# epam/ai-dial-rag

Hardware: AMD Instinct MI355X
Metric: retrieval_qps_10Mx384 (higher is better)
Workload: dtype f32 (int8 MFMA filter with exact integer dot products and a rigorous error margin, every candidate the margin cannot exclude re-scored in f64 with the reference formula)

## Files before the change

ai-dial-rag_amd/csrc/vec_kernels.h:

```cpp
#pragma once
#include <hip/hip_runtime.h>
#include <stdint.h>

#include <type_traits>

namespace mir {

typedef __attribute__((ext_vector_type(8))) __bf16 bf16x8;
typedef __attribute__((ext_vector_type(16))) float f32x16;

constexpr int kTileRows = 32;
constexpr int kMaxList = 64;
constexpr int kListMargin = 8;
constexpr int kSortN = 8192;
constexpr double kScanSplitErr = 4.6e-5;
__host__ __device__ constexpr double scan_rel_err(int d) { return kScanSplitErr + 6.0e-8 * (d < 384 ? 384 : d); }

enum ScanKind { SCAN_IP = 0, SCAN_L2 = 1, SCAN_COS = 2 };


__device__ __forceinline__ uint32_t bf16_rne_bits(float x) {
    uint32_t u = __float_as_uint(x);
    if ((u & 0x7fffffffu) > 0x7f800000u) return 0x7fc0u;
    return (u + 0x7fffu + ((u >> 16) & 1u)) >> 16;
// ... 131 lines not shown
}

__device__ __forceinline__ float ref_row_norm(double s, float doc_sq32) {
    return doc_sq32 == __builtin_inff() ? __builtin_inff() : fmaxf((float)sqrt(s), 1e-8f);
}

template <typename T>
__global__ __launch_bounds__(256) void row_norms_kernel(const T *__restrict__ src, int64_t n, int d,
                                                        float *__restrict__ doc_sq,
                                                        float *__restrict__ inv_norm,
                                                        unsigned int *__restrict__ max_norm_bits) {
    int64_t row = (int64_t)blockIdx.x * 256 + threadIdx.x;
    float nrm = 0.f, res = 0.f, rel = 0.f;
    if (row < n) {
        const T *a = src + row * (int64_t)d;
        const float dsq = np_pairwise_sq<12>(a, d);
        doc_sq[row] = dsq;
        const double s = seq_sum_sq_f64(a, d);
        nrm = (float)sqrt(s);
        nrm = nrm * (1.0f + 1e-6f);
        inv_norm[row] = 1.0f / ref_row_norm(s, dsq);
        if (sizeof(T) == 4) {
            res = bf16_residual_norm(a, d);
            rel = res * inv_norm[row] * (1.0f + 1e-6f);
        }
    }
    for (int off = 32; off >= 1; off >>= 1) { res = fmaxf(res, __shfl_xor(res, off, 64)); rel = fmaxf(rel, __shfl_xor(rel, off, 64)); }
    if ((threadIdx.x & 63) == 0 && res > 0.f) { atomicMax(max_norm_bits + 2, __float_as_uint(res)); atomicMax(max_norm_bits + 3, __float_as_uint(rel)); }
    if (__ballot(!(nrm < __builtin_inff())) != 0ull && (threadIdx.x & 63) == 0) atomicOr(max_norm_bits + 1, 1u);
    for (int off = 32; off >= 1; off >>= 1) nrm = fmaxf(nrm, __shfl_xor(nrm, off, 64));
    if ((threadIdx.x & 63) == 0 && nrm > 0.f) atomicMax(max_norm_bits, __float_as_uint(nrm));
}

constexpr int kNormsLdsBytes = 64 * 1024;
__host__ __device__ inline int norms_row_stride(int d) { return d | 1; }
template <typename T>
__global__ __launch_bounds__(256) void row_norms_lds_kernel(const T *__restrict__ src, int64_t n, int d, int rows_per_wg,
                                                            float *__restrict__ doc_sq, float *__restrict__ inv_norm,
                                                            unsigned int *__restrict__ max_norm_bits) {
    extern __shared__ float norms_lds[];
    const int stride = norms_row_stride(d);
    const int64_t row0 = (int64_t)blockIdx.x * rows_per_wg;
    const int rows = (int)(n - row0 < rows_per_wg ? n - row0 : rows_per_wg);
    const T *base = src + row0 * (int64_t)d;
    const int total = rows * d;
    for (int e0 = threadIdx.x; e0 < total; e0 += 256 * 16) {
        T v[16];
#pragma unroll
        for (int u = 0; u < 16; ++u) {
            const int e = e0 + 256 * u;
            v[u] = e < total ? base[e] : T(0);
        }
        int r = e0 / d, c = e0 - r * d;
#pragma unroll
        for (int u = 0; u < 16; ++u) {
            if (e0 + 256 * u < total) norms_lds[r * stride + c] = (float)v[u];
            c += 256;
            while (c >= d) { c -= d; ++r; }
        }
    }
    __syncthreads();
    float nrm = 0.f, res = 0.f, rel = 0.f;
    const int rt = threadIdx.x & 127;
    const float *a = norms_lds + rt * stride;
    const int64_t row = row0 + rt;
    double s = 0.0;
    if (rt < rows) {
        if (threadIdx.x < 128) {
            doc_sq[row] = np_pairwise_sq<12>(a, d);
        } else {
            s = seq_sum_sq_f64(a, d);
        }
    }
    __syncthreads();
    if (rt < rows && threadIdx.x >= 128) {
        nrm = (float)sqrt(s);
        nrm = nrm * (1.0f + 1e-6f);
        inv_norm[row] = 1.0f / ref_row_norm(s, const_cast<const volatile float *>(doc_sq)[row]);
        if (sizeof(T) == 4) {
            res = bf16_residual_norm(a, d);
            rel = res * inv_norm[row] * (1.0f + 1e-6f);
        }
    }
    for (int off = 32; off >= 1; off >>= 1) { res = fmaxf(res, __shfl_xor(res, off, 64)); rel = fmaxf(rel, __shfl_xor(rel, off, 64)); }
    if ((threadIdx.x & 63) == 0 && res > 0.f) { atomicMax(max_norm_bits + 2, __float_as_uint(res)); atomicMax(max_norm_bits + 3, __float_as_uint(rel)); }
    if (__ballot(!(nrm < __builtin_inff())) != 0ull && (threadIdx.x & 63) == 0) atomicOr(max_norm_bits + 1, 1u);
    for (int off = 32; off >= 1; off >>= 1) nrm = fmaxf(nrm, __shfl_xor(nrm, off, 64));
    if ((threadIdx.x & 63) == 0 && nrm > 0.f) atomicMax(max_norm_bits, __float_as_uint(nrm));
}


__global__ __launch_bounds__(64) void prep_queries_kernel(const double *__restrict__ q, int b, int d, int ksteps,
                                                          int ngroups, uint4 *__restrict__ qsplit,
                                                          double *__restrict__ q_sq,
                                                          double *__restrict__ q_norm,
                                                          unsigned long long *__restrict__ gthr, int gthr_words) {
    int lane = threadIdx.x;
    int blk = blockIdx.x;
    if (gthr && blk * 64 + lane < gthr_words) gthr[blk * 64 + lane] = 0;
    if (blk < ngroups * ksteps) {
        int s = blk % ksteps;
        int g = blk / ksteps;
        int qi = 32 * g + (lane & 31);
        int col0 = 16 * s + 8 * (lane >> 5);
        uint32_t hi[8], lo[8];
#pragma unroll
        for (int j = 0; j < 8; ++j) {
            float x = (qi < b && col0 + j < d) ? (float)q[(int64_t)qi * d + col0 + j] : 0.f;
            split_bf16(x, hi[j], lo[j]);
        }
        qsplit[((int64_t)blk * 2 + 0) * 64 + lane] = pack8(hi);
        qsplit[((int64_t)blk * 2 + 1) * 64 + lane] = pack8(lo);
    } else {
        int qi = blk - ngroups * ksteps;
        if (qi >= b) return;
        double s = 0.0;
        for (int j = lane; j < d; j += 64) {
            double x = q[(int64_t)qi * d + j];
            s += x * x;
        }
        s = wave_sum(s);
        if (lane == 0) {
            q_sq[qi] = s;
            q_norm[qi] = sqrt(s);
        }
    }
}


template <int STRIDE = 256>
__device__ __forceinline__ void list_insert(uint64_t *list, int klist, int tid, uint64_t key, uint64_t &minkey,
                                            int &minpos) {
    list[minpos * STRIDE + tid] = key;
    uint64_t m = ~0ull;
    int mp = 0;
    for (int p0 = 0; p0 < klist; p0 += 8) {
        uint64_t x[8];
#pragma unroll
        for (int j = 0; j < 8; ++j) x[j] = (p0 + j < klist) ? list[(p0 + j) * STRIDE + tid] : ~0ull;
#pragma unroll
        for (int j = 0; j < 8; ++j) {
            if (x[j] < m) {
                m = x[j];
                mp = p0 + j;
            }
        }
    }
    minkey = m;
    minpos = mp;
}

template <int KIND>
__device__ __forceinline__ void tile_epilogue(const f32x16 &acc_m, const f32x16 &acc_c, const float4 (&ax)[4],
                                              uint32_t row0, uint32_t n_rows, uint64_t *list, int klist, int tid,
                                              uint64_t &minkey, int &minpos) {
    float v[16];
    uint32_t mask = 0;
    const float vmin = key_value(minkey);
    const bool open = minkey == 0;
#pragma unroll
    for (int r = 0; r < 16; ++r) {
        const int g = r >> 2, i = r & 3;
        const float dot = acc_m[r] + acc_c[r];
        float x;
        if (KIND == SCAN_IP) {
            x = dot;
        } else {
            const float a = (i == 0) ? ax[g].x : (i == 1) ? ax[g].y : (i == 2) ? ax[g].z : ax[g].w;
            x = (KIND == SCAN_L2) ? fmaf(2.0f, dot, -a) : dot * a;
        }
        x = (x == x) ? x + 0.0f : -__builtin_inff();
        v[r] = x;
        const uint32_t row = row0 + 8 * g + i;
        if (row < n_rows && (open || x >= vmin)) mask |= 1u << r;
    }
    while (mask) {
        const int r = __builtin_ctz(mask);
        mask &= mask - 1;
        float x = v[0];
#pragma unroll
        for (int j = 1; j < 16; ++j) x = (r == j) ? v[j] : x;
        const uint32_t row = row0 + 8 * (r >> 2) + (r & 3);
        const uint64_t key = make_key(x, row);
        if (key > minkey) list_insert(list, klist, tid, key, minkey, minpos);
    }
}

template <int KSTEPS, int KIND>
__global__ __launch_bounds__(256, 1) void scan_topk_kernel(const uint4 *__restrict__ docs,
                                                           const float *__restrict__ aux,
                                                           const uint4 *__restrict__ qsplit, uint32_t n_rows,
                                                           uint32_t n_tiles, int nq, int klist,
                                                           uint64_t *__restrict__ part) {
    extern __shared__ __attribute__((aligned(16))) unsigned char smem[];
    uint64_t *list = reinterpret_cast<uint64_t *>(smem);
    uint64_t *stage = list + klist * 256;

    constexpr int R = KSTEPS < 8 ? KSTEPS : 8;
    static_assert(KSTEPS % R == 0, "ring slot must be static across tiles");
    constexpr int TILE_U4 = KSTEPS * 128;

    const int tid = threadIdx.x;
    const int lane = tid & 63;
    const int h = lane >> 5;
    const int qj = lane & 31;
    const uint32_t wave_global = blockIdx.x * 4 + (tid >> 6);
    const uint32_t total_waves = gridDim.x * 4;

    for (int p = 0; p < klist; ++p) list[p * 256 + tid] = 0;
    uint64_t minkey = 0;
    int minpos = 0;

    if (wave_global < n_tiles) {
        bf16x8 qh[KSTEPS], ql[KSTEPS];
#pragma unroll
        for (int s = 0; s < KSTEPS; ++s) {
            qh[s] = __builtin_bit_cast(bf16x8, qsplit[(s * 2 + 0) * 64 + lane]);
            ql[s] = __builtin_bit_cast(bf16x8, qsplit[(s * 2 + 1) * 64 + lane]);
        }

        uint32_t t = wave_global;
        const uint4 *tp = docs + (size_t)t * TILE_U4 + lane;
        uint4 bh[R], bl[R];
#pragma unroll
        for (int i = 0; i < R; ++i) {
            bh[i] = tp[(2 * i + 0) * 64];
            bl[i] = tp[(2 * i + 1) * 64];
        }

        while (true) {
            const uint32_t tn = t + total_waves;
            const bool more = tn < n_tiles;
            const uint4 *np = docs + (size_t)(more ? tn : t) * TILE_U4 + lane;

            float4 ax[4];
            if (KIND != SCAN_IP) {
                const float4 *ap = reinterpret_cast<const float4 *>(aux + (size_t)t * kTileRows);
#pragma unroll
                for (int g = 0; g < 4; ++g) ax[g] = ap[2 * g + h];
            }

            f32x16 acc_m = {0}, acc_c = {0};
#pragma unroll
            for (int ks = 0; ks < KSTEPS; ++ks) {
                const int slot = ks % R;
                bf16x8 ah = __builtin_bit_cast(bf16x8, bh[slot]);
                bf16x8 al = __builtin_bit_cast(bf16x8, bl[slot]);
                acc_m = __builtin_amdgcn_mfma_f32_32x32x16_bf16(ah, qh[ks], acc_m, 0, 0, 0);
                acc_c = __builtin_amdgcn_mfma_f32_32x32x16_bf16(ah, ql[ks], acc_c, 0, 0, 0);
                acc_c = __builtin_amdgcn_mfma_f32_32x32x16_bf16(al, qh[ks], acc_c, 0, 0, 0);
                if (ks + R < KSTEPS) {
                    bh[slot] = tp[(2 * (ks + R) + 0) * 64];
                    bl[slot] = tp[(2 * (ks + R) + 1) * 64];
                } else {
                    bh[slot] = np[(2 * (ks + R - KSTEPS) + 0) * 64];
                    bl[slot] = np[(2 * (ks + R - KSTEPS) + 1) * 64];
                }
                __builtin_amdgcn_sched_barrier(0);
            }

            if (qj < nq) tile_epilogue<KIND>(acc_m, acc_c, ax, t * kTileRows + 4 * h, n_rows, list, klist, tid, minkey, minpos);
            if (!more) break;
            t = tn;
            tp = np;
        }
    }

    __syncthreads();
    for (int i = tid; i < 32 * klist; i += 256) stage[i] = 0;
    __syncthreads();
    for (int p = 0; p < klist; ++p) {
        const uint64_t key = list[p * 256 + tid];
        if (key == 0) continue;
        int rank = 0;
        for (int l = 0; l < 8; ++l) {
            const int t2 = 64 * (l >> 1) + 32 * (l & 1) + qj;
            for (int p2 = 0; p2 < klist; ++p2) rank += (list[p2 * 256 + t2] > key) ? 1 : 0;
        }
        if (rank < klist) stage[qj * klist + rank] = key;
    }
    __syncthreads();
    uint64_t *out = part + (size_t)blockIdx.x * 32 * klist;
    for (int i = tid; i < 32 * klist; i += 256) out[i] = stage[i];
}

constexpr int kB128Pending = 4;

__device__ __forceinline__ void glds16_b128(const void *gsrc, uint32_t lds_byte_addr) {
    uint32_t keep;
    asm volatile(
        "s_mov_b32 %0, m0\n\ts_mov_b32 m0, %2\n\ts_nop 0\n\tglobal_load_lds_dwordx4 %1, off nt\n\ts_mov_b32 m0, %0"
        : "=&s"(keep)
        : "v"(gsrc), "s"(lds_byte_addr)
        : "memory");
}
__device__ __forceinline__ void glds4_b32(const void *gsrc, uint32_t lds_byte_addr) {
    uint32_t keep;
    asm volatile(
        "s_mov_b32 %0, m0\n\ts_mov_b32 m0, %2\n\ts_nop 0\n\tglobal_load_lds_dword %1, off\n\ts_mov_b32 m0, %0"
        : "=&s"(keep)
        : "v"(gsrc), "s"(lds_byte_addr)
        : "memory");
}
__device__ __forceinline__ void glds4_b32_sv(const void *gbase_uniform, uint32_t lane_byte_off, uint32_t lds_byte_addr) {
    uint32_t keep;
    asm volatile(
        "s_mov_b32 %0, m0\n\ts_mov_b32 m0, %3\n\ts_nop 0\n\tglobal_load_lds_dword %1, %2\n\ts_mov_b32 m0, %0"
        : "=&s"(keep)
        : "v"(lane_byte_off), "s"(gbase_uniform), "s"(lds_byte_addr)
        : "memory");
}
__device__ __forceinline__ uint32_t lds_addr_of(const void *p) {
    return (uint32_t)(uintptr_t)(const __attribute__((address_space(3))) void *)p;
}

template <int STRIDE = 256>
__device__ __forceinline__ void drain_candidates(uint32_t mask, const float (&v)[16], uint32_t row0, uint64_t *list,
                                                 int klist, int tid, uint64_t &minkey, int &minpos, int &pending) {
    while (__any(mask != 0)) {
        if (mask) {
            const int r = __builtin_ctz(mask);
            mask &= mask - 1;
            float x = v[0];
#pragma unroll
            for (int j = 1; j < 16; ++j) {
                float c = v[j];
                asm volatile("" : "+v"(c));
                x = (r == j) ? c : x;
            }
            x = (x == x) ? x + 0.0f : -__builtin_inff();
            const uint64_t key = make_key(x, row0 + 8 * (r >> 2) + (r & 3));
            if (key > minkey) {
                list[(klist + pending) * STRIDE + tid] = key;
                ++pending;
            }
        }
        if (__any(pending == kB128Pending)) {
            for (int i = 0; i < kB128Pending; ++i) {
                if (i < pending) {
                    const uint64_t key = list[(klist + i) * STRIDE + tid];
                    if (key > minkey) list_insert<STRIDE>(list, klist, tid, key, minkey, minpos);
                }
            }
            pending = 0;
        }
    }
}

template <int KIND>
__global__ __launch_bounds__(256, 1) void scan_topk_generic_kernel(const uint4 *__restrict__ docs,
                                                                   const float *__restrict__ aux,
                                                                   const uint4 *__restrict__ qsplit,
                                                                   int ksteps, uint32_t n_rows,
                                                                   uint32_t n_tiles, int nq, int klist,
                                                                   uint64_t *__restrict__ part) {
    extern __shared__ __attribute__((aligned(16))) unsigned char smem[];
    uint64_t *list = reinterpret_cast<uint64_t *>(smem);
    uint64_t *stage = list + klist * 256;
    constexpr int R = 8;
    const size_t tile_u4 = (size_t)ksteps * 128;
    const int tid = threadIdx.x, lane = tid & 63, h = lane >> 5, qj = lane & 31;
    const uint32_t wave_global = blockIdx.x * 4 + (tid >> 6);
    const uint32_t total_waves = gridDim.x * 4;
    for (int p = 0; p < klist; ++p) list[p * 256 + tid] = 0;
    uint64_t minkey = 0;
    int minpos = 0;

    for (uint32_t t = wave_global; t < n_tiles; t += total_waves) {
        const uint4 *tp = docs + (size_t)t * tile_u4 + lane;
        const uint4 *qp = qsplit + lane;
        float4 ax[4];
        if (KIND != SCAN_IP) {
            const float4 *ap = reinterpret_cast<const float4 *>(aux + (size_t)t * kTileRows);
#pragma unroll
            for (int g = 0; g < 4; ++g) ax[g] = ap[2 * g + h];
        }
        f32x16 acc_m = {0}, acc_c = {0};
        for (int k0 = 0; k0 < ksteps; k0 += R) {
            uint4 dh[R], dl[R], qh[R], ql[R];
#pragma unroll
            for (int i = 0; i < R; ++i) {
                dh[i] = tp[(2 * (k0 + i) + 0) * 64];
                dl[i] = tp[(2 * (k0 + i) + 1) * 64];
                qh[i] = qp[(2 * (k0 + i) + 0) * 64];
                ql[i] = qp[(2 * (k0 + i) + 1) * 64];
            }
#pragma unroll
            for (int i = 0; i < R; ++i) {
                bf16x8 ah = __builtin_bit_cast(bf16x8, dh[i]), al = __builtin_bit_cast(bf16x8, dl[i]);
                bf16x8 bh = __builtin_bit_cast(bf16x8, qh[i]), bl = __builtin_bit_cast(bf16x8, ql[i]);
                acc_m = __builtin_amdgcn_mfma_f32_32x32x16_bf16(ah, bh, acc_m, 0, 0, 0);
                acc_c = __builtin_amdgcn_mfma_f32_32x32x16_bf16(ah, bl, acc_c, 0, 0, 0);
                acc_c = __builtin_amdgcn_mfma_f32_32x32x16_bf16(al, bh, acc_c, 0, 0, 0);
            }
        }
        if (qj < nq) tile_epilogue<KIND>(acc_m, acc_c, ax, t * kTileRows + 4 * h, n_rows, list, klist, tid, minkey, minpos);
    }
    __syncthreads();
    for (int i = tid; i < 32 * klist; i += 256) stage[i] = 0;
    __syncthreads();
    for (int p = 0; p < klist; ++p) {
        const uint64_t key = list[p * 256 + tid];
        if (key == 0) continue;
        int rank = 0;
        for (int l = 0; l < 8; ++l) {
            const int t2 = 64 * (l >> 1) + 32 * (l & 1) + qj;
            for (int p2 = 0; p2 < klist; ++p2) rank += (list[p2 * 256 + t2] > key) ? 1 : 0;
        }
        if (rank < klist) stage[qj * klist + rank] = key;
    }
    __syncthreads();
    uint64_t *out = part + (size_t)blockIdx.x * 32 * klist;
    for (int i = tid; i < 32 * klist; i += 256) out[i] = stage[i];
}


template <typename T, int W = 64, int U = 8>
__device__ __forceinline__ double exact_metric_wave(const T *__restrict__ row, const double *__restrict__ q,
                                                    int d, int metric, float doc_sq32, double q_sq,
                                                    double q_norm, int lane, double *rank_value) {
    if (metric == MIR_METRIC_COSINE_SIM) {
        double s = 0.0;
        for (int j0 = lane; j0 < d; j0 += W * U) {
            float v[U];
#pragma unroll
            for (int u = 0; u < U; ++u) v[u] = j0 + W * u < d ? (float)row[j0 + W * u] : 0.f;
#pragma unroll
            for (int u = 0; u < U; ++u)
                if (j0 + W * u < d) {
                    const double x = (double)v[u];
                    s += x * x;
                }
        }
        s = group_sum<W>(s);
        const float dn = ref_row_norm(s, doc_sq32);
        const double qn = fmax(q_norm, 1e-8);
        double c = 0.0;
        for (int j0 = lane; j0 < d; j0 += W * U) {
            float v[U];
            double qv[U];
#pragma unroll
            for (int u = 0; u < U; ++u) {
                const bool in = j0 + W * u < d;
                v[u] = in ? (float)row[j0 + W * u] : 0.f;
                qv[u] = in ? q[j0 + W * u] : 0.0;
            }
#pragma unroll
            for (int u = 0; u < U; ++u)
                if (j0 + W * u < d) c += (double)__fdiv_rn(v[u], dn) * (qv[u] / qn);
        }
        c = group_sum<W>(c);
        *rank_value = c * qn;
        return -c;
    }
    double dot = 0.0;
    for (int j0 = lane; j0 < d; j0 += W * U) {
        float v[U];
        double qv[U];
#pragma unroll
        for (int u = 0; u < U; ++u) {
            const bool in = j0 + W * u < d;
            v[u] = in ? (float)row[j0 + W * u] : 0.f;
            qv[u] = in ? q[j0 + W * u] : 0.0;
        }
#pragma unroll
        for (int u = 0; u < U; ++u)
            if (j0 + W * u < d) dot += (double)v[u] * qv[u];
    }
    dot = group_sum<W>(dot);
    if (metric == MIR_METRIC_INNER_PRODUCT) {
        *rank_value = dot;
        return -dot;
    }
    const double sq = ((double)doc_sq32 - 2.0 * dot) + q_sq;
    *rank_value = 2.0 * dot - (double)doc_sq32;
    return metric == MIR_METRIC_SQEUCLIDEAN_DIST ? sq : sqrt(sq);
}

__device__ __forceinline__ bool dist_before(double da, uint32_t ra, double db, uint32_t rb) {
    const bool na = da != da, nb = db != db;
    if (na || nb) return na == nb ? ra < rb : nb;
    return da < db || (da == db && ra < rb);
}

template <typename T>
__global__ __launch_bounds__(256) void metric_eval_kernel(const T *__restrict__ docs,
                                                          const float *__restrict__ doc_sq, int64_t n, int d,
                                                          const double *__restrict__ q,
                                                          const double *__restrict__ q_sq,
                                                          const double *__restrict__ q_norm, int metric,
                                                          double *__restrict__ out) {
    const int lane = threadIdx.x & 63;
    const int64_t row = (int64_t)blockIdx.x * 4 + (threadIdx.x >> 6);
    if (row >= n) return;
    double rv;
    double dist = exact_metric_wave(docs + row * (int64_t)d, q, d, metric, doc_sq[row], q_sq[0], q_norm[0], lane, &rv);
    if (lane == 0) out[row] = dist;
}


__device__ inline void bitonic_sort_desc(uint64_t *keys, int n, int tid) {
    for (int size = 2; size <= n; size <<= 1) {
        for (int stride = size >> 1; stride > 0; stride >>= 1) {
            __syncthreads();
            for (int i = tid; i < (n >> 1); i += 256) {
                const int lo = 2 * i - (i & (stride - 1));
                const int hi = lo + stride;
                const bool desc = (lo & size) == 0;
                const uint64_t a = keys[lo], b = keys[hi];
                if ((a < b) == desc) {
                    keys[lo] = b;
                    keys[hi] = a;
                }
            }
        }
    }
    __syncthreads();
}

__device__ inline void merge_sorted_lists(const uint64_t *__restrict__ lists, size_t list_stride, int nwg, int klist,
                                          uint64_t *out, uint64_t *red , int tid) {
    int head[4];
    uint64_t cur[4], n1[4], n2[4];
#pragma unroll
    for (int j = 0; j < 4; ++j) {
        const int wg = tid + 256 * j;
        const bool mine_j = wg < nwg;
        const uint64_t *l = lists + (size_t)wg * list_stride;
        head[j] = 0;
        cur[j] = mine_j ? l[0] : 0;
        n1[j] = (mine_j && klist > 1) ? l[1] : 0;
        n2[j] = (mine_j && klist > 2) ? l[2] : 0;
    }
    for (int r = 0; r < klist; ++r) {
        uint64_t mine = cur[0];
#pragma unroll
        for (int j = 1; j < 4; ++j) mine = cur[j] > mine ? cur[j] : mine;
        uint64_t best = mine;
#pragma unroll
        for (int off = 32; off >= 1; off >>= 1) {
            const uint64_t o = ((uint64_t)__shfl_xor((uint32_t)(best >> 32), off, 64) << 32) |
                               (uint64_t)__shfl_xor((uint32_t)best, off, 64);
            best = o > best ? o : best;
        }
        if ((tid & 63) == 0) red[tid >> 6] = best;
        __syncthreads();
        best = red[0];
#pragma unroll
        for (int w = 1; w < 4; ++w) best = red[w] > best ? red[w] : best;
        __syncthreads();
        if (tid == 0) out[r] = best;
        if (best != 0 && mine == best) {
#pragma unroll
            for (int j = 0; j < 4; ++j) {
                if (cur[j] == best) {
                    ++head[j];
                    if (head[j] == 1) cur[j] = n1[j];
                    else if (head[j] == 2) cur[j] = n2[j];
                    else cur[j] = head[j] < klist ? lists[(size_t)(tid + 256 * j) * list_stride + head[j]] : 0;
                }
            }
        }
    }
    __syncthreads();
}

constexpr int kXbCols = 192;
constexpr int kXbQ = 128;
__host__ __device__ constexpr int xb_dpad(int d) { return (d + kXbCols - 1) / kXbCols * kXbCols; }
__device__ __forceinline__ void exact_publish_query(double *__restrict__ qt, int f, const double *__restrict__ q, int d, int metric,
                                                    double q_norm, int tid, int nthreads) {
    const int dpad = xb_dpad(d);
    const double qn = fmax(q_norm, 1e-8);
    double *dst = qt + ((size_t)(f / kXbQ) * dpad) * kXbQ + (f % kXbQ);
    for (int j = tid; j < dpad; j += nthreads) {
        double x = j < d ? q[j] : 0.0;
        if (metric == MIR_METRIC_COSINE_SIM) x = x / qn;
        dst[(size_t)j * kXbQ] = x;
    }
}

__device__ __forceinline__ bool query_filterable(bool l2, double qn, float max_norm) {
    if (qn == 0.0) return true;
    if (!(qn >= 0x1p-100 && qn <= 0x1p100)) return false;
    return !(l2 && qn > 0x1p24 * (double)max_norm);
}

struct FinalizeArgs {
    const uint64_t *part;
    int nwg;
    int qpw;
    int klist;
    int k;
    int b;
    int d;
    int metric;
    const float *docs;
    const _Float16 *docs16;
    const float *doc_sq;
    const float *max_norm;
    double scan_rel_err;
    const double *q;
    const double *q_sq;
    const double *q_norm;
    const int64_t *chunk_ids;
    const int32_t *doc_ids;
    int64_t row_offset;
    int32_t *out_doc;
    int64_t *out_chunk;
    int64_t *out_row;
    double *out_dist;
    int32_t *out_count;
    int32_t *out_flags;
// ... 399 lines not shown
```

ai-dial-rag_amd/csrc/vec_kernels_i8.h:

```cpp
#pragma once
#include "vec_kernels_sieve.h"

#ifndef I8_ABL
#define I8_ABL 0
#endif

namespace mir {

typedef int __attribute__((ext_vector_type(4))) i32x4;

constexpr int kI8StatWords = 8;
constexpr int kI8MaxK = 16;
static_assert(kI8MaxK <= kSieveSampleMaxK, "the exact sample threshold evaluates k rows in one round");
constexpr int kI8Region = 32768;
constexpr int kI8WavePart = kI8Region / 8;
__device__ __forceinline__ void i8_margin_ab(float qn, float eq, const float *__restrict__ stats, float &A, float &B) {
    i8_margin_ab_decl(qn, eq, stats, A, B);
}
__device__ __forceinline__ float i8_margin_tile(bool l2, float A, float B, float e_t, float s_t, float sq) {
    const float m = fmaf(e_t, A, B) + 2.0f * s_t * sq;
    return l2 ? 2.0f * m : m;
}

__global__ __launch_bounds__(256) void i8_tile_scale_kernel(const float *__restrict__ src, int64_t n, int d, float4 *__restrict__ tparam) {
    __shared__ float red[4];
    const int64_t tile = blockIdx.x;
    const int64_t r0 = tile * kTileRows;
    const int64_t rows = n - r0 < kTileRows ? n - r0 : kTileRows;
    const float *p = src + r0 * (int64_t)d;
    float m = 0.f;
    for (int64_t i = threadIdx.x; i < rows * d; i += 256) m = fmaxf(m, fabsf(p[i]));
#pragma unroll
    for (int off = 32; off >= 1; off >>= 1) m = fmaxf(m, __shfl_xor(m, off, 64));
    if ((threadIdx.x & 63) == 0) red[threadIdx.x >> 6] = m;
    __syncthreads();
    if (threadIdx.x == 0) {
        m = fmaxf(fmaxf(red[0], red[1]), fmaxf(red[2], red[3]));
        const float st = m > 0.f ? m / 127.0f : 1.0f;
        tparam[tile] = make_float4(st, 0.f, 0.5f / st, 0.f);
    }
}
__global__ void i8_scale_kernel(float *__restrict__ stats, const float *__restrict__ max_norm) {
    stats[0] = max_norm[0];
    stats[7] = __builtin_inff();
}

__device__ __forceinline__ int i8_quant(float x, float inv) {
    const float r = rintf(x * inv);
    return (int)fminf(fmaxf(r, -127.0f), 127.0f);
}

__global__ __launch_bounds__(256) void pack_i8_kernel(const float *__restrict__ src, int64_t n, int d, int ks64, int64_t total_lanes,
                                                      const float4 *__restrict__ tparam, uint4 *__restrict__ dst) {
    const int64_t gid = (int64_t)blockIdx.x * 256 + threadIdx.x;
    if (gid >= total_lanes) return;
    const int lane = (int)(gid & 63);
    const int64_t blk = gid >> 6;
    const int nb = ks64 * 2;
    const int b = (int)(blk % nb);
    const int64_t tile = blk / nb;
    const int s = b >> 1, rh = b & 1;
    const int64_t row = tile * kTileRows + 16 * rh + (lane & 15);
    const int col0 = 64 * s + 16 * (lane >> 4);
    uint32_t w[4] = {0u, 0u, 0u, 0u};
    if (row < n) {
        const float inv = 1.0f / tparam[tile].x;
#pragma unroll
        for (int j = 0; j < 16; ++j) {
            const float x = col0 + j < d ? src[row * (int64_t)d + col0 + j] : 0.f;
            w[j >> 2] |= ((uint32_t)i8_quant(x, inv) & 0xffu) << (8 * (j & 3));
        }
    }
    dst[blk * 64 + lane] = make_uint4(w[0], w[1], w[2], w[3]);
}

__global__ __launch_bounds__(256) void i8_residual_kernel(const float *__restrict__ src, int64_t n, int d, const float *__restrict__ doc_sq,
                                                          float4 *__restrict__ tparam, float *__restrict__ stats) {
    const int lg = threadIdx.x & 15;
    const int64_t row = (int64_t)blockIdx.x * 16 + (threadIdx.x >> 4);
    double e2 = 0.0;
    if (row < n) {
        const float s = tparam[row / kTileRows].x;
        const float inv = 1.0f / s;
        for (int j = lg; j < d; j += 16) {
            const float x = src[row * (int64_t)d + j];
            const double r = (double)x - (double)s * (double)i8_quant(x, inv);
            e2 += r * r;
        }
    }
    e2 = group_sum<16>(e2);
    if (lg == 0 && row < n) {
        const float e = (float)sqrt(e2) * (1.0f + 1e-6f);
        atomicMax(reinterpret_cast<unsigned int *>(&tparam[row / kTileRows].y), __float_as_uint(e));
        const float a = doc_sq[row];
        const volatile float *vs = stats;
        if (e > vs[2]) atomicMax(reinterpret_cast<unsigned int *>(stats) + 2, __float_as_uint(e));
        if (a > vs[1]) atomicMax(reinterpret_cast<unsigned int *>(stats) + 1, __float_as_uint(a));
        if (a < vs[7]) atomicMin(reinterpret_cast<unsigned int *>(stats) + 7, __float_as_uint(a));
    }
}

__global__ __launch_bounds__(128) void i8_stage_record_kernel(const float *__restrict__ col, int64_t n_col, const float4 *__restrict__ tparam,
                                                              float *__restrict__ rec) {
    const int64_t stage = blockIdx.x;
    const int t = threadIdx.x;
    if (t >= 72) return;
    float v;
    if (t < 64) {
        const int64_t row = stage * 64 + t;
        v = row < n_col ? col[row] : 0.f;
    } else {
        v = reinterpret_cast<const float *>(tparam)[stage * 8 + (t - 64)];
    }
    rec[stage * 72 + t] = v;
}

__global__ __launch_bounds__(64) void prep_queries_i8_stats_kernel(const double *__restrict__ q, int b, int d, double *__restrict__ q_sq,
                                                                   double *__restrict__ q_norm, float *__restrict__ q_amax,
                                                                   unsigned long long *__restrict__ gthr, int gthr_words) {
    const int lane = threadIdx.x, blk = blockIdx.x;
    if (gthr && blk * 64 + lane < gthr_words) gthr[blk * 64 + lane] = 0;
    const int qi = blk;
    if (qi >= b) return;
    double s = 0.0;
    float m = 0.f;
    bool bad = false;
    for (int j = lane; j < d; j += 64) {
        const double x = q[(int64_t)qi * d + j];
        s += x * x;
        const float a = fabsf((float)x);
        bad |= !(a < __builtin_inff());
        m = fmaxf(m, a);
    }
    s = wave_sum(s);
#pragma unroll
    for (int off = 32; off >= 1; off >>= 1) m = fmaxf(m, __shfl_xor(m, off, 64));
    bad = __any(bad);
    if (lane == 0) {
        q_sq[qi] = s;
        q_norm[qi] = sqrt(s);
        q_amax[qi] = bad ? -1.0f : m;
    }
}
__global__ __launch_bounds__(64) void prep_queries_i8_quant_kernel(const double *__restrict__ q, int b, int d, int ks64, int ntiles16,
                                                                   const float *__restrict__ q_amax, uint4 *__restrict__ qfrag,
                                                                   double *__restrict__ q_err, float *__restrict__ q_scale) {
    const int lane = threadIdx.x, blk = blockIdx.x;
    if (blk < ntiles16 * ks64) {
        const int s = blk % ks64, w = blk / ks64;
        const int qi = 16 * w + (lane & 15);
        const int col0 = 64 * s + 16 * (lane >> 4);
        uint32_t wv[4] = {0u, 0u, 0u, 0u};
        const float m = qi < b ? q_amax[qi] : -1.0f;
        if (m >= 0.f) {
            const float inv = m > 0.f ? 127.0f / m : 1.0f;
#pragma unroll
            for (int j = 0; j < 16; ++j) {
                const float x = col0 + j < d ? (float)q[(int64_t)qi * d + col0 + j] : 0.f;
                wv[j >> 2] |= ((uint32_t)i8_quant(x, inv) & 0xffu) << (8 * (j & 3));
            }
        }
        qfrag[(int64_t)blk * 64 + lane] = make_uint4(wv[0], wv[1], wv[2], wv[3]);
    } else {
        const int qi = blk - ntiles16 * ks64;
        if (qi >= b) return;
        const float m = q_amax[qi];
        const bool ok = m >= 0.f;
        const float inv = m > 0.f ? 127.0f / m : 1.0f;
        const float sq = 1.0f / inv;
        double e2 = 0.0;
        for (int j = lane; j < d; j += 64) {
            const double x = q[(int64_t)qi * d + j];
            const double r = ok ? x - (double)sq * (double)i8_quant((float)x, inv) : x;
            e2 += r * r;
        }
        e2 = wave_sum(e2);
        if (lane == 0) {
            q_err[qi] = sqrt(e2);
            q_scale[qi] = sq;
        }
    }
}

__host__ __device__ constexpr int sieve_i8_stages(int nw) { return nw == 8 ? kSieveStages : 3; }
__host__ __device__ constexpr size_t sieve_i8_lds_bytes(int ks64, int nw) { return (size_t)sieve_i8_stages(nw) * (ks64 * 4 * 1024 + (64 + 8) * 4) + 64; }

template <int KS64, int KIND, bool SAMPLE, int QT, int NW>
__global__ __launch_bounds__(NW * 64, 2) void sieve_i8_kernel(const uint4 *__restrict__ docs, const float *__restrict__ aux,
                                                          const uint4 *__restrict__ qfrag, const double *__restrict__ q_norm,
                                                          const double *__restrict__ q_sq, const double *__restrict__ q_err,
                                                          const float *__restrict__ stats, const float *__restrict__ q_scale,
                                                          uint32_t n_rows, uint32_t stage0, uint32_t n_stages, int nq, int nan_guard,
                                                          const uint64_t *__restrict__ gthr, uint64_t *__restrict__ cand,
                                                          float *__restrict__ candv, uint32_t *__restrict__ ccount,
                                                          float *__restrict__ part_sample, unsigned long long *__restrict__ stat) {
    static_assert(KIND == SCAN_L2 || KIND == SCAN_IP || KIND == SCAN_COS, "scan kind");
    static_assert(QT == 1 || QT == 2 || QT == 4, "query tiles per wave");
    static_assert(NW == 8 || NW == 4, "waves per workgroup");
    constexpr int NS = sieve_i8_stages(NW);
    constexpr int APW = 64 / NW;
    constexpr int NB = KS64 * 2;
    constexpr int SB = NB * 2;
    constexpr int STAGE_U4 = SB * 64;
    constexpr int PPW = SB / NW;
    constexpr int PW = PPW + 1;
    constexpr int AS = 64 + 8;
    constexpr int D = NS - 1;
    constexpr int QPL = NW * 16 * QT;
    static_assert(SB % NW == 0, "sieve_i8: d padded to a multiple of 128");
    extern __shared__ __attribute__((aligned(16))) unsigned char smem[];
    uint4 *ring = reinterpret_cast<uint4 *>(smem);
    float *aux_lds = reinterpret_cast<float *>(smem + (size_t)NS * STAGE_U4 * 16);

    const int tid = threadIdx.x, lane = tid & 63, qc = lane & 15, jg = lane >> 4;
    const int wave8 = __builtin_amdgcn_readfirstlane(tid >> 6);
    const uint32_t G = gridDim.x;

    const float amin = KIND == SCAN_L2 ? stats[7] : 0.f;
    int qloc[QT];
    bool lane_live[QT];
    unsigned long long live_mask[QT];
    constexpr float L = KIND == SCAN_L2 ? 2.0f : 1.0f;
    const float ax_hi = KIND == SCAN_COS ? stats[6] : 1.0f;
    float tbc[QT];
    float sq[QT], mA[QT], mB[QT], P1[QT], A1[QT], guard[QT], best[QT];
    uint32_t brow[QT];
    i32x4 qh[QT][KS64];
    const bool active = nq > wave8 * QT * 16;
#pragma unroll
    for (int u = 0; u < QT; ++u) {
        const int t16 = wave8 * QT + u;
        qloc[u] = t16 * 16 + qc;
        lane_live[u] = qloc[u] < nq && (SAMPLE || query_filterable(KIND == SCAN_L2, q_norm[qloc[u]], stats[0]));
        live_mask[u] = __builtin_amdgcn_ballot_w64(lane_live[u]);
        sq[u] = 1.0f; mA[u] = 0.f; mB[u] = 0.f; P1[u] = -__builtin_inff(); A1[u] = 0.f; tbc[u] = -__builtin_inff();
        guard[u] = __builtin_inff(); best[u] = -__builtin_inff(); brow[u] = 0;
        if (lane_live[u]) {
            const float qn = (float)q_norm[qloc[u]] * (1.0f + 1e-6f);
            const float eq = (float)q_err[qloc[u]] * (1.0f + 1e-6f);
            const bool good = qn < __builtin_inff() && eq < __builtin_inff();
            sq[u] = q_scale[qloc[u]];
            if (good) i8_margin_ab(qn, eq, stats, mA[u], mB[u]);
            if (!SAMPLE) {
                const uint64_t key = gthr[qloc[u]];
                if (key != 0 && good) {
                    const float t = key_value(key);
                    float tb = t - 2e-6f * fabsf(t);
                    tbc[u] = tb;
                    if (KIND == SCAN_COS) tb = fminf(tb * stats[4], tb * stats[5]) - 1e-6f * fabsf(tb) * stats[5];
                    P1[u] = (tb + amin - L * mB[u]) / (L * sq[u]);
                    A1[u] = mA[u] / sq[u];
                    if (!(P1[u] == P1[u]) || !(A1[u] == A1[u])) { P1[u] = -__builtin_inff(); A1[u] = 0.f; tbc[u] = -__builtin_inff(); }
                }
            } else if (nan_guard) {
                const float qs = (float)q_sq[qloc[u]];
                guard[u] = qs - 1e-5f * fabsf(qs);
            }
        }
        const uint4 *qs = qfrag + (size_t)t16 * KS64 * 64 + lane;
#pragma unroll
        for (int s = 0; s < KS64; ++s) qh[u][s] = __builtin_bit_cast(i32x4, qs[s * 64]);
    }
    const uint32_t my_stages = blockIdx.x < n_stages ? (n_stages - blockIdx.x + G - 1) / G : 0;
    const uint32_t NG = my_stages;

    auto issue = [&](uint32_t g) {
        const uint32_t stage = stage0 + blockIdx.x + g * G;
        const uint4 *src = docs + (size_t)stage * STAGE_U4 + (wave8 * PPW) * 64 + lane;
        const uint32_t dst = __builtin_amdgcn_readfirstlane(lds_addr_of(ring) + ((g % NS) * STAGE_U4 + (wave8 * PPW) * 64) * 16);
#pragma unroll
        for (int i = 0; i < PPW; ++i) glds16_b128(src + i * 64, dst + i * 1024);
        {
            const uint32_t adst = __builtin_amdgcn_readfirstlane(lds_addr_of(aux_lds) + ((g % NS) * AS + wave8 * APW) * 4);
            const float *abase = aux + (size_t)stage * AS + wave8 * APW;
            if (lane < APW + (wave8 == NW - 1 ? 8 : 0)) glds4_b32_sv(abase, (uint32_t)lane * 4u, adst);
        }
    };
#pragma unroll
    for (int u = 0; u < QT; ++u)
#pragma unroll
        for (int s = 0; s < KS64; ++s) asm volatile("" : "+v"(qh[u][s]));
    asm volatile("s_waitcnt vmcnt(0)" ::: "memory");
    for (uint32_t g = 0; g < (uint32_t)D && g < NG; ++g) issue(g);

    auto wait_stage = [&](uint32_t g) {
        const uint32_t younger = (NG - 1 - g) < (uint32_t)(D - 1) ? (NG - 1 - g) : (uint32_t)(D - 1);
        if (younger == (uint32_t)(D - 1)) asm volatile("s_waitcnt vmcnt(%0)" ::"i"((D - 1) * PW) : "memory");
        else asm volatile("s_waitcnt vmcnt(0)" ::: "memory");
    };
    uint64_t *region = cand + ((size_t)blockIdx.x * NW + wave8) * kI8WavePart;
    float *regionv = candv + ((size_t)blockIdx.x * NW + wave8) * kI8WavePart;
    const unsigned long long lt_mask = (1ull << lane) - 1ull;
    uint32_t wcount = 0;

    auto filter = [&](int u, const i32x4 &c0, const i32x4 &c1, const float (&ax)[8], uint32_t t, const float4 &tp) {
        if (SAMPLE) {
            if (lane_live[u]) {
                const float vs = L * tp.x * sq[u], mg = i8_margin_tile(KIND == SCAN_L2, mA[u], mB[u], tp.y, tp.x, sq[u]) * ax_hi;
#pragma unroll
                for (int r = 0; r < 8; ++r) {
                    const float fi = (float)(r < 4 ? c0[r & 3] : c1[r & 3]);
                    const float w = KIND == SCAN_L2 ? fmaf(vs, fi, -ax[r]) : KIND == SCAN_COS ? vs * fi * ax[r] : vs * fi;
                    const uint32_t row = t * kTileRows + 4 * jg + 16 * (r >> 2) + (r & 3);
                    if (w + mg < guard[u] && w - mg > best[u] && row < n_rows) { best[u] = w - mg; brow[u] = row; }
                }
            }
            return;
        }
        const float x2 = fmaf(fmaf(-tp.y, A1[u], P1[u]), 2.0f * tp.z, -4.0f);
        const int ib = (int)__builtin_amdgcn_fmed3f(floorf(x2), -2.0e9f, 2.0e9f);
        const int m0 = max(max(c0[0], c0[1]), c0[2]), m1 = max(max(c0[3], c1[0]), c1[1]);
        const int m = max(max(max(c1[2], c1[3]), m0), m1);
        if ((__builtin_amdgcn_ballot_w64(m >= ib) & live_mask[u]) == 0ull) return;
        asm volatile("" : "+s"(t));
        const float vs = L * tp.x * sq[u];
        float bound = (fmaf(-tp.y, A1[u], P1[u]) - 2.0f * tp.x) * (L * sq[u]) - amin;
        if (KIND == SCAN_COS) bound = tbc[u] - i8_margin_tile(false, mA[u], mB[u], tp.y, tp.x, sq[u]) * ax_hi;
        const float bound_w = bound - 4e-6f * (fabsf(bound) + amin);
        float v[8];
#pragma unroll
        for (int r = 0; r < 8; ++r) {
            const float fi = (float)(r < 4 ? c0[r & 3] : c1[r & 3]);
            v[r] = KIND == SCAN_L2 ? fmaf(vs, fi, -ax[r]) : KIND == SCAN_COS ? vs * fi * ax[r] : vs * fi;
        }
        uint32_t pm = 0;
#pragma unroll
        for (int r = 0; r < 8; ++r) pm |= (uint32_t)(!(v[r] < bound_w)) << r;
        if (!lane_live[u]) pm = 0;
        if (!__any(pm != 0)) return;
        const uint32_t row0 = t * kTileRows + 4 * jg;
        if (t * kTileRows + kTileRows > n_rows) {
#pragma unroll
            for (int r = 0; r < 8; ++r)
                if (row0 + 16 * (r >> 2) + (r & 3) >= n_rows) pm &= ~(1u << r);
        }
        while (__any(pm != 0)) {
            const bool has = pm != 0;
            const int r = has ? __builtin_ctz(pm) : 0;
            const unsigned long long bal = __ballot(has);
            const uint32_t slot = wcount + (uint32_t)__popcll(bal & lt_mask);
            wcount += (uint32_t)__popcll(bal);
            float vr = v[0];
#pragma unroll
            for (int i = 1; i < 8; ++i) vr = r == i ? v[i] : vr;
            if (has && slot < (uint32_t)kI8WavePart) {
                region[slot] = ((uint64_t)(uint32_t)qloc[u] << 32) | (uint64_t)(row0 + 16 * (r >> 2) + (r & 3));
                regionv[slot] = vr;
            }
            pm &= pm - 1;
        }
    };

    i32x4 p0[QT], p1[QT];
#pragma unroll
    for (int u = 0; u < QT; ++u) { p0[u] = i32x4{0, 0, 0, 0}; p1[u] = i32x4{0, 0, 0, 0}; }
    float pax[8] = {};
    float4 ptp = make_float4(1.f, 0.f, 0.5f, 0.f);
    uint32_t pt = 0;
    bool have_prev = false;
    for (uint32_t g = 0; g < my_stages; ++g) {
        const uint32_t stage = stage0 + blockIdx.x + g * G;
#if !(I8_ABL & 4)
        wait_stage(g);
#endif
#if !(I8_ABL & 2)
        __builtin_amdgcn_s_barrier();
#endif
        if (!active) {
            if (g + D < NG) issue(g + D);
            continue;
        }
#pragma unroll
        for (int sub = 0; sub < 2; ++sub) {
            const uint4 *st = ring + (size_t)(g % NS) * STAGE_U4 + sub * (NB * 64) + lane;
            constexpr int PF = QT == 4 ? 1 : (2 < KS64 ? 2 : KS64 - 1);
            uint4 f0[PF + 1], f1[PF + 1];
#pragma unroll
            for (int i = 0; i < PF; ++i) { f0[i] = st[(2 * i + 0) * 64]; f1[i] = st[(2 * i + 1) * 64]; }
            const float4 ctp = *reinterpret_cast<const float4 *>(aux_lds + (g % NS) * AS + 64 + 4 * sub);
            float cax[8] = {};
            if (KIND != SCAN_IP) {
                const float4 a0 = *reinterpret_cast<const float4 *>(aux_lds + (g % NS) * AS + 32 * sub + 4 * jg);
                const float4 a1 = *reinterpret_cast<const float4 *>(aux_lds + (g % NS) * AS + 32 * sub + 16 + 4 * jg);
                cax[0] = a0.x; cax[1] = a0.y; cax[2] = a0.z; cax[3] = a0.w;
                cax[4] = a1.x; cax[5] = a1.y; cax[6] = a1.z; cax[7] = a1.w;
            }
            i32x4 c0[QT], c1[QT];
#pragma unroll
            for (int u = 0; u < QT; ++u) { c0[u] = i32x4{0, 0, 0, 0}; c1[u] = i32x4{0, 0, 0, 0}; }
#pragma unroll
            for (int s = 0; s < KS64; ++s) {
                if (s + PF < KS64) {
                    f0[(s + PF) % (PF + 1)] = st[(2 * (s + PF) + 0) * 64];
                    f1[(s + PF) % (PF + 1)] = st[(2 * (s + PF) + 1) * 64];
                }
                __builtin_amdgcn_sched_barrier(0);
#pragma unroll
                for (int u = 0; u < QT; ++u) {
                    c0[u] = __builtin_amdgcn_mfma_i32_16x16x64_i8(__builtin_bit_cast(i32x4, f0[s % (PF + 1)]), qh[u][s], c0[u], 0, 0, 0);
                    c1[u] = __builtin_amdgcn_mfma_i32_16x16x64_i8(__builtin_bit_cast(i32x4, f1[s % (PF + 1)]), qh[u][s], c1[u], 0, 0, 0);
                }
                if (sub == 0 && s == 0) {
                    __builtin_amdgcn_sched_barrier(0);
#if !(I8_ABL & 4)
                    if (g + D < NG) issue(g + D);
#endif
                }
#pragma unroll
                for (int u = 0; u < QT; ++u)
                    if (s == 1 + u && s < KS64 && have_prev) {
                        __builtin_amdgcn_sched_barrier(0);
#if I8_ABL & 1
                        if (g == 0xffffff)
#endif
                        filter(u, p0[u], p1[u], pax, pt, ptp);
                    }
            }
            if (KS64 < QT + 1 && have_prev) {
#pragma unroll
                for (int u = KS64 - 1; u < QT; ++u) filter(u, p0[u], p1[u], pax, pt, ptp);
            }
#pragma unroll
            for (int u = 0; u < QT; ++u) { p0[u] = c0[u]; p1[u] = c1[u]; }
#pragma unroll
            for (int i = 0; i < 8; ++i) pax[i] = cax[i];
            ptp = ctp;
            pt = stage * 2 + sub;
            have_prev = true;
        }
    }
    if (have_prev) {
#pragma unroll
        for (int u = 0; u < QT; ++u) filter(u, p0[u], p1[u], pax, pt, ptp);
    }
    if (SAMPLE) {
        uint32_t *part_row = reinterpret_cast<uint32_t *>(part_sample + (size_t)gridDim.x * QPL * 2);
#pragma unroll
        for (int u = 0; u < QT; ++u) {
            const float o = __shfl_xor(best[u], 16, 64);
            const uint32_t orow = (uint32_t)__shfl_xor((int)brow[u], 16, 64);
            const bool other = o > best[u];
            const float b2 = other ? o : best[u];
            const size_t at = ((size_t)blockIdx.x * QPL + qloc[u]) * 2 + (jg >> 1);
            if (lane_live[u] && (jg == 0 || jg == 2)) {
                part_sample[at] = b2;
                part_row[at] = other ? orow : brow[u];
            }
        }
        return;
    }
    if (lane == 0) {
        ccount[(size_t)blockIdx.x * NW + wave8] = wcount;
        if (stat && wcount) atomicAdd(stat, (unsigned long long)wcount);
    }
}

__global__ __launch_bounds__(256) void sieve_scatter_i8_kernel(SieveScatterArgs a) {
    __shared__ uint32_t s_cnt[256], s_base[256];
    const int tid = threadIdx.x;
    const int part = blockIdx.x;
    uint32_t cnt = a.ccount[part];
    s_cnt[tid] = 0;
    __syncthreads();
    if (cnt > (uint32_t)kI8WavePart) {
        for (int i = tid; i < a.nq; i += 256) a.l.over[a.q0 + i] = 1;
        cnt = kI8WavePart;
    }
    const uint64_t *region = a.cand + (size_t)part * kI8WavePart;
    const float *regionv = a.candv + (size_t)part * kI8WavePart;
    for (uint32_t e = tid; e < cnt; e += 256) atomicAdd(&s_cnt[(int)(region[e] >> 32) & 255], 1u);
    __syncthreads();
    {
        const uint32_t c = s_cnt[tid];
        s_base[tid] = c ? atomicAdd(&a.l.count[(size_t)(a.q0 + tid) * kSieveCountStride], c) : 0u;
        s_cnt[tid] = 0;
    }
    __syncthreads();
    for (uint32_t e = tid; e < cnt; e += 256) {
        const uint64_t key = region[e];
        const int ql = (int)(key >> 32) & 255, qi = a.q0 + ql;
        const uint32_t slot = s_base[ql] + atomicAdd(&s_cnt[ql], 1u);
        if (slot < (uint32_t)kSieveQueryCap) {
            a.l.row[(size_t)qi * kSieveQueryCap + slot] = (uint32_t)key;
            a.l.rv[(size_t)qi * kSieveQueryCap + slot] = regionv[e];
        } else {
            a.l.over[qi] = 1;
        }
    }
}

}
```

Measured before the change: 247,500.

## Batch stage DMA into one asm block and interleave filter VALU under MFMAs

Stage loads now go out as a single inline-asm sequence per wave: immediate offsets on global_load_lds_dwordx4 plus an exec-masked dword load for the aux record, using incrementing pointers and slot counters in place of per-stage address recomputation. The filter threshold check becomes a float compare against a precomputed 2*z term, which drops the floor/med3/convert work. The filter also uses sched_group_barrier so its VALU work is interleaved with the MFMA stream instead of being fenced by a sched_barrier. The have_prev flag is removed by initialising the previous tile with a sentinel so the first filter pass is harmless, which relies on that sentinel behaving correctly.

Result: slower. 229,200 (-7.4%).

```diff
diff --git a/ai-dial-rag_amd/csrc/vec_kernels.h b/ai-dial-rag_amd/csrc/vec_kernels.h
--- a/ai-dial-rag_amd/csrc/vec_kernels.h
+++ b/ai-dial-rag_amd/csrc/vec_kernels.h
@@ -457,13 +457,36 @@
         : "v"(gsrc), "s"(lds_byte_addr)
         : "memory");
 }
-__device__ __forceinline__ void glds4_b32_sv(const void *gbase_uniform, uint32_t lane_byte_off, uint32_t lds_byte_addr) {
-    uint32_t keep;
-    asm volatile(
-        "s_mov_b32 %0, m0\n\ts_mov_b32 m0, %3\n\ts_nop 0\n\tglobal_load_lds_dword %1, %2\n\ts_mov_b32 m0, %0"
-        : "=&s"(keep)
-        : "v"(lane_byte_off), "s"(gbase_uniform), "s"(lds_byte_addr)
-        : "memory");
+template <int PPW>
+__device__ __forceinline__ void glds_stage(uint32_t lane_off, const void *gbase, const void *gbase4k, uint32_t lds_dst,
+                                           uint32_t lds_dst4k, const void *rec_base, uint32_t rec_lds_dst, uint64_t rec_lanes) {
+    static_assert(PPW == 1 || PPW == 2 || PPW == 3 || PPW == 4 || PPW == 6, "glds_stage: pieces per wave");
+    uint32_t keep, rec_lane_off;
+#define MIR_GLDS_HEAD "s_mov_b32 %0, m0\n\ts_mov_b32 m0, %4\n\ts_nop 0\n\t"
+#define MIR_GLDS_PIECE(off) "global_load_lds_dwordx4 %2, %3 offset:" #off " nt\n\t"
+#define MIR_GLDS_PIECE4K(off) "global_load_lds_dwordx4 %2, %8 offset:" #off " nt\n\t"
+#define MIR_GLDS_REC "s_mov_b32 m0, %6\n\ts_mov_b64 exec, %7\n\tv_lshrrev_b32 %1, 2, %2\n\tglobal_load_lds_dword %1, %5\n\ts_mov_b64 exec, -1\n\ts_mov_b32 m0, %0"
+#define MIR_GLDS_OPS : "=&s"(keep), "=&v"(rec_lane_off) : "v"(lane_off), "s"(gbase), "s"(lds_dst), "s"(rec_base), "s"(rec_lds_dst), "s"(rec_lanes)
+    if constexpr (PPW == 1) {
+        asm volatile(MIR_GLDS_HEAD MIR_GLDS_PIECE(0) MIR_GLDS_REC MIR_GLDS_OPS : "memory");
+    } else if constexpr (PPW == 2) {
+        asm volatile(MIR_GLDS_HEAD MIR_GLDS_PIECE(0) MIR_GLDS_PIECE(1024) MIR_GLDS_REC MIR_GLDS_OPS : "memory");
+    } else if constexpr (PPW == 3) {
+        asm volatile(MIR_GLDS_HEAD MIR_GLDS_PIECE(0) MIR_GLDS_PIECE(1024) MIR_GLDS_PIECE(2048) MIR_GLDS_REC MIR_GLDS_OPS : "memory");
+    } else if constexpr (PPW == 4) {
+        asm volatile(MIR_GLDS_HEAD MIR_GLDS_PIECE(0) MIR_GLDS_PIECE(1024) MIR_GLDS_PIECE(2048) MIR_GLDS_PIECE(3072) MIR_GLDS_REC MIR_GLDS_OPS
+                     : "memory");
+    } else {
+        asm volatile(MIR_GLDS_HEAD MIR_GLDS_PIECE(0) MIR_GLDS_PIECE(1024) MIR_GLDS_PIECE(2048) MIR_GLDS_PIECE(3072)
+                     "s_mov_b32 m0, %9\n\ts_nop 0\n\t" MIR_GLDS_PIECE4K(0) MIR_GLDS_PIECE4K(1024) MIR_GLDS_REC MIR_GLDS_OPS,
+                     "s"(gbase4k), "s"(lds_dst4k)
+                     : "memory");
+    }
+#undef MIR_GLDS_HEAD
+#undef MIR_GLDS_PIECE
+#undef MIR_GLDS_PIECE4K
+#undef MIR_GLDS_REC
+#undef MIR_GLDS_OPS
 }
 __device__ __forceinline__ uint32_t lds_addr_of(const void *p) {
     return (uint32_t)(uintptr_t)(const __attribute__((address_space(3))) void *)p;
diff --git a/ai-dial-rag_amd/csrc/vec_kernels_i8.h b/ai-dial-rag_amd/csrc/vec_kernels_i8.h
--- a/ai-dial-rag_amd/csrc/vec_kernels_i8.h
+++ b/ai-dial-rag_amd/csrc/vec_kernels_i8.h
@@ -8,6 +8,7 @@
 namespace mir {
 
 typedef int __attribute__((ext_vector_type(4))) i32x4;
+typedef __attribute__((address_space(3))) i32x4 lds_u4;
 
 constexpr int kI8StatWords = 8;
 constexpr int kI8MaxK = 16;
@@ -184,6 +185,20 @@
 
 __host__ __device__ constexpr int sieve_i8_stages(int nw) { return nw == 8 ? kSieveStages : 3; }
 __host__ __device__ constexpr size_t sieve_i8_lds_bytes(int ks64, int nw) { return (size_t)sieve_i8_stages(nw) * (ks64 * 4 * 1024 + (64 + 8) * 4) + 64; }
+
+struct I8TileParam { float x, y, z2; };
+template <int N_MFMA, int VPM>
+__device__ __forceinline__ void mfma_shadow() {
+#if I8_ABL & 8
+    __builtin_amdgcn_sched_barrier(0);
+#else
+#pragma unroll
+    for (int i = 0; i < N_MFMA; ++i) {
+        __builtin_amdgcn_sched_group_barrier(0x008, 1, 0);
+        __builtin_amdgcn_sched_group_barrier(0x002, VPM, 0);
+    }
+#endif
+}
 
 template <int KS64, int KIND, bool SAMPLE, int QT, int NW>
 __global__ __launch_bounds__(NW * 64, 2) void sieve_i8_kernel(const uint4 *__restrict__ docs, const float *__restrict__ aux,
@@ -264,24 +279,27 @@
     const uint32_t my_stages = blockIdx.x < n_stages ? (n_stages - blockIdx.x + G - 1) / G : 0;
     const uint32_t NG = my_stages;
 
-    auto issue = [&](uint32_t g) {
-        const uint32_t stage = stage0 + blockIdx.x + g * G;
-        const uint4 *src = docs + (size_t)stage * STAGE_U4 + (wave8 * PPW) * 64 + lane;
-        const uint32_t dst = __builtin_amdgcn_readfirstlane(lds_addr_of(ring) + ((g % NS) * STAGE_U4 + (wave8 * PPW) * 64) * 16);
-#pragma unroll
-        for (int i = 0; i < PPW; ++i) glds16_b128(src + i * 64, dst + i * 1024);
-        {
-            const uint32_t adst = __builtin_amdgcn_readfirstlane(lds_addr_of(aux_lds) + ((g % NS) * AS + wave8 * APW) * 4);
-            const float *abase = aux + (size_t)stage * AS + wave8 * APW;
-            if (lane < APW + (wave8 == NW - 1 ? 8 : 0)) glds4_b32_sv(abase, (uint32_t)lane * 4u, adst);
-        }
+    constexpr uint32_t STAGE_BYTES = STAGE_U4 * 16;
+    const uint32_t dma_lane_off = (uint32_t)lane * 16u;
+    const uint64_t rec_lanes = (1ull << (APW + (wave8 == NW - 1 ? 8 : 0))) - 1ull;
+    const uint32_t ring_dst = __builtin_amdgcn_readfirstlane(lds_addr_of(ring) + (wave8 * PPW) * 1024);
+    const uint32_t rec_dst = __builtin_amdgcn_readfirstlane(lds_addr_of(aux_lds) + (wave8 * APW) * 4);
+    const char *isrc = reinterpret_cast<const char *>(docs) + (size_t)(stage0 + blockIdx.x) * STAGE_BYTES + (wave8 * PPW) * 1024;
+    const float *irec = aux + (size_t)(stage0 + blockIdx.x) * AS + wave8 * APW;
+    uint32_t islot = 0;
+    auto issue = [&]() {
+        glds_stage<PPW>(dma_lane_off, isrc, isrc + 4096, ring_dst + islot * STAGE_BYTES, ring_dst + islot * STAGE_BYTES + 4096, irec,
+                        rec_dst + islot * (AS * 4), rec_lanes);
+        isrc += (size_t)G * STAGE_BYTES;
+        irec += (size_t)G * AS;
+        islot = islot + 1 == (uint32_t)NS ? 0u : islot + 1;
     };
 #pragma unroll
     for (int u = 0; u < QT; ++u)
 #pragma unroll
         for (int s = 0; s < KS64; ++s) asm volatile("" : "+v"(qh[u][s]));
     asm volatile("s_waitcnt vmcnt(0)" ::: "memory");
-    for (uint32_t g = 0; g < (uint32_t)D && g < NG; ++g) issue(g);
+    for (uint32_t g = 0; g < (uint32_t)D && g < NG; ++g) issue();
 
     auto wait_stage = [&](uint32_t g) {
         const uint32_t younger = (NG - 1 - g) < (uint32_t)(D - 1) ? (NG - 1 - g) : (uint32_t)(D - 1);
@@ -293,7 +311,8 @@
     const unsigned long long lt_mask = (1ull << lane) - 1ull;
     uint32_t wcount = 0;
 
-    auto filter = [&](int u, const i32x4 &c0, const i32x4 &c1, const float (&ax)[8], uint32_t t, const float4 &tp) {
+    auto filter = [&](auto shadow, int u, const i32x4 &c0, const i32x4 &c1, const float (&ax)[8], uint32_t t, const I8TileParam &tp) {
+        constexpr bool SHADOW = decltype(shadow)::value;
         if (SAMPLE) {
             if (lane_live[u]) {
                 const float vs = L * tp.x * sq[u], mg = i8_margin_tile(KIND == SCAN_L2, mA[u], mB[u], tp.y, tp.x, sq[u]) * ax_hi;
@@ -305,13 +324,15 @@
                     if (w + mg < guard[u] && w - mg > best[u] && row < n_rows) { best[u] = w - mg; brow[u] = row; }
                 }
             }
+            if (SHADOW) mfma_shadow<2 * QT, 8 / QT>();
             return;
         }
-        const float x2 = fmaf(fmaf(-tp.y, A1[u], P1[u]), 2.0f * tp.z, -4.0f);
-        const int ib = (int)__builtin_amdgcn_fmed3f(floorf(x2), -2.0e9f, 2.0e9f);
+        const float xb = fmaf(fmaf(-tp.y, A1[u], P1[u]), tp.z2, -6.0f);
         const int m0 = max(max(c0[0], c0[1]), c0[2]), m1 = max(max(c0[3], c1[0]), c1[1]);
         const int m = max(max(max(c1[2], c1[3]), m0), m1);
-        if ((__builtin_amdgcn_ballot_w64(m >= ib) & live_mask[u]) == 0ull) return;
+        const bool pass = !((float)m < xb);
+        if (SHADOW) mfma_shadow<2 * QT, 4 / QT>();
+        if ((__builtin_amdgcn_ballot_w64(pass) & live_mask[u]) == 0ull) return;
         asm volatile("" : "+s"(t));
         const float vs = L * tp.x * sq[u];
         float bound = (fmaf(-tp.y, A1[u], P1[u]) - 2.0f * tp.x) * (L * sq[u]) - amin;
@@ -355,11 +376,11 @@
 #pragma unroll
     for (int u = 0; u < QT; ++u) { p0[u] = i32x4{0, 0, 0, 0}; p1[u] = i32x4{0, 0, 0, 0}; }
     float pax[8] = {};
-    float4 ptp = make_float4(1.f, 0.f, 0.5f, 0.f);
-    uint32_t pt = 0;
-    bool have_prev = false;
+    I8TileParam ptp = {1.f, 0.f, 1.f};
+    uint32_t pt = 0x07fffffeu;
+    uint32_t cslot = 0;
+    uint32_t ctile = (stage0 + blockIdx.x) * 2;
     for (uint32_t g = 0; g < my_stages; ++g) {
-        const uint32_t stage = stage0 + blockIdx.x + g * G;
 #if !(I8_ABL & 4)
         wait_stage(g);
 #endif
@@ -367,21 +388,24 @@
         __builtin_amdgcn_s_barrier();
 #endif
         if (!active) {
-            if (g + D < NG) issue(g + D);
+            if (g + D < NG) issue();
             continue;
         }
+        const lds_u4 *sring = reinterpret_cast<const lds_u4 *>((uintptr_t)(lds_addr_of(ring) + cslot * STAGE_BYTES + dma_lane_off));
+        const float *srec = aux_lds + cslot * AS;
 #pragma unroll
         for (int sub = 0; sub < 2; ++sub) {
-            const uint4 *st = ring + (size_t)(g % NS) * STAGE_U4 + sub * (NB * 64) + lane;
+            const lds_u4 *st = sring + sub * (NB * 64);
             constexpr int PF = QT == 4 ? 1 : (2 < KS64 ? 2 : KS64 - 1);
-            uint4 f0[PF + 1], f1[PF + 1];
+            i32x4 f0[PF + 1], f1[PF + 1];
 #pragma unroll
             for (int i = 0; i < PF; ++i) { f0[i] = st[(2 * i + 0) * 64]; f1[i] = st[(2 * i + 1) * 64]; }
-            const float4 ctp = *reinterpret_cast<const float4 *>(aux_lds + (g % NS) * AS + 64 + 4 * sub);
+            const float2 cxy = *reinterpret_cast<const float2 *>(srec + 64 + 4 * sub);
+            const float cz = srec[64 + 4 * sub + 2];
             float cax[8] = {};
             if (KIND != SCAN_IP) {
-                const float4 a0 = *reinterpret_cast<const float4 *>(aux_lds + (g % NS) * AS + 32 * sub + 4 * jg);
-                const float4 a1 = *reinterpret_cast<const float4 *>(aux_lds + (g % NS) * AS + 32 * sub + 16 + 4 * jg);
+                const float4 a0 = *reinterpret_cast<const float4 *>(srec + 32 * sub + 4 * jg);
+                const float4 a1 = *reinterpret_cast<const float4 *>(srec + 32 * sub + 16 + 4 * jg);
                 cax[0] = a0.x; cax[1] = a0.y; cax[2] = a0.z; cax[3] = a0.w;
                 cax[4] = a1.x; cax[5] = a1.y; cax[6] = a1.z; cax[7] = a1.w;
             }
@@ -397,41 +421,41 @@
                 __builtin_amdgcn_sched_barrier(0);
 #pragma unroll
                 for (int u = 0; u < QT; ++u) {
-                    c0[u] = __builtin_amdgcn_mfma_i32_16x16x64_i8(__builtin_bit_cast(i32x4, f0[s % (PF + 1)]), qh[u][s], c0[u], 0, 0, 0);
-                    c1[u] = __builtin_amdgcn_mfma_i32_16x16x64_i8(__builtin_bit_cast(i32x4, f1[s % (PF + 1)]), qh[u][s], c1[u], 0, 0, 0);
+                    c0[u] = __builtin_amdgcn_mfma_i32_16x16x64_i8(f0[s % (PF + 1)], qh[u][s], c0[u], 0, 0, 0);
+                    c1[u] = __builtin_amdgcn_mfma_i32_16x16x64_i8(f1[s % (PF + 1)], qh[u][s], c1[u], 0, 0, 0);
                 }
                 if (sub == 0 && s == 0) {
                     __builtin_amdgcn_sched_barrier(0);
 #if !(I8_ABL & 4)
-                    if (g + D < NG) issue(g + D);
+                    if (g + D < NG) issue();
 #endif
                 }
 #pragma unroll
                 for (int u = 0; u < QT; ++u)
-                    if (s == 1 + u && s < KS64 && have_prev) {
-                        __builtin_amdgcn_sched_barrier(0);
+                    if (s == 1 + u && s < KS64) {
 #if I8_ABL & 1
                         if (g == 0xffffff)
 #endif
-                        filter(u, p0[u], p1[u], pax, pt, ptp);
+                        filter(std::true_type{}, u, p0[u], p1[u], pax, pt, ptp);
                     }
             }
-            if (KS64 < QT + 1 && have_prev) {
-#pragma unroll
-                for (int u = KS64 - 1; u < QT; ++u) filter(u, p0[u], p1[u], pax, pt, ptp);
+            if (KS64 < QT + 1) {
+#pragma unroll
+                for (int u = KS64 - 1; u < QT; ++u) filter(std::false_type{}, u, p0[u], p1[u], pax, pt, ptp);
             }
 #pragma unroll
             for (int u = 0; u < QT; ++u) { p0[u] = c0[u]; p1[u] = c1[u]; }
 #pragma unroll
             for (int i = 0; i < 8; ++i) pax[i] = cax[i];
-            ptp = ctp;
-            pt = stage * 2 + sub;
-            have_prev = true;
-        }
-    }
-    if (have_prev) {
-#pragma unroll
-        for (int u = 0; u < QT; ++u) filter(u, p0[u], p1[u], pax, pt, ptp);
+            ptp = I8TileParam{cxy.x, cxy.y, 2.0f * cz};
+            pt = ctile + sub;
+        }
+        cslot = cslot + 1 == (uint32_t)NS ? 0u : cslot + 1;
+        ctile += 2 * G;
+    }
+    if (my_stages != 0 && active) {
+#pragma unroll
+        for (int u = 0; u < QT; ++u) filter(std::false_type{}, u, p0[u], p1[u], pax, pt, ptp);
     }
     if (SAMPLE) {
         uint32_t *part_row = reinterpret_cast<uint32_t *>(part_sample + (size_t)gridDim.x * QPL * 2);
```
